# mohsij/spacecraft-pose-estimation

Hardware: AMD Instinct MI355X
Metric: poses/sec end-to-end (HRNet+PnP) at batch 256; keypoint/pose err vs ref (higher is better)
Workload: dtype bf16

## Files before the change

spacecraft-pose-estimation_amd/csrc/common.h:

```cpp
#pragma once
#include <hip/hip_runtime.h>
#include <stdint.h>
#include <stddef.h>
#include <stdarg.h>
#include <stdio.h>
#include <string>
#include <vector>
#include <string.h>

#include "../../include/scpose.h"

namespace scpose {

void set_error(const char* fmt, ...);
const char* dev_env(const char* name);
const char* last_error();

#define SCP_CHECK_HIP(expr)                                                         \
  do {                                                                              \
    hipError_t _e = (expr);                                                         \
    if (_e != hipSuccess) {                                                         \
      ::scpose::set_error("%s failed: %s (%s:%d)", #expr, hipGetErrorString(_e),    \
                          __FILE__, __LINE__);                                      \
      return SCPOSE_E_HIP;                                                          \
    }                                                                               \
  } while (0)

#define SCP_REQUIRE(cond, ...)            \
  do {                                    \
    if (!(cond)) {                        \
      ::scpose::set_error(__VA_ARGS__);   \
      return SCPOSE_E_INVALID;            \
    }                                     \
  } while (0)

#ifdef SCPOSE_DEV_BUILD
#define SCP_DBG(p, bits) ((p).dbg & (bits))
#define SCP_DBG_BUF(p) ((p).dbg_buf)
#define SCP_DEV_ONLY(x) (x)
constexpr bool kDevBuild = true;
#else
#define SCP_DBG(p, bits) (0)
#define SCP_DBG_BUF(p) (static_cast<unsigned long long*>(nullptr))
#define SCP_DEV_ONLY(x) (0)
constexpr bool kDevBuild = false;
#endif

struct LdsOptIn {
  bool done[16] = {false};
};
int32_t lds_opt_in(const void* kernel, int bytes, LdsOptIn* memo);

struct FastDiv {
  uint32_t mul, shift, add, d;
};
inline FastDiv make_fastdiv(uint32_t d) {
  FastDiv f; f.d = d ? d : 1;
  uint32_t s = 0;
  while ((2u << s) <= f.d) ++s;
  if ((f.d & (f.d - 1)) == 0) { f.mul = 0; f.add = 1; f.shift = s; }
  else { f.mul = (uint32_t)((((uint64_t)1 << (32 + s)) / f.d) + 1); f.add = 0; f.shift = s; }
  return f;
}

inline size_t align256(size_t b) { return (b + 255) & ~(size_t)255; }
struct Carve {
  uint8_t* base;
  size_t off = 0;
  template <class T>
  T* take(size_t count) {
    T* p = base ? reinterpret_cast<T*>(base + off) : nullptr;
    off += align256(count * sizeof(T));
    return p;
  }
  size_t bytes() const { return off; }
};

constexpr size_t kBufLimit = 0xfffffff0ull;
inline size_t blocked_bytes(int n, int planes, int h, int w) { return (size_t)n * planes * h * w * 16; }
inline bool fits_buf(size_t bytes) { return bytes < kBufLimit; }
inline int buf_max_frames(size_t frame_bytes, int cap = 0) {
  const int max_n = (int)(kBufLimit / frame_bytes);
  return cap > 0 && cap < max_n ? cap : max_n;
}
struct FrameRangeSwitches { int cap; bool print; };
const FrameRangeSwitches& frame_range_switches();
template <class Launch>
__attribute__((format(printf, 4, 5))) int32_t for_frame_ranges(int N, size_t frame_bytes, Launch&& launch, const char* name_fmt, ...) {
  const FrameRangeSwitches& sw = frame_range_switches();
  char name[96] = "";
  if (sw.print || !fits_buf(frame_bytes)) {
    va_list ap;
    va_start(ap, name_fmt);
    vsnprintf(name, sizeof(name), name_fmt, ap);
    va_end(ap);
  }
  SCP_REQUIRE(fits_buf(frame_bytes), "%s: one frame (%zu bytes) does not fit a 32-bit buffer descriptor", name, frame_bytes);
  const int max_n = buf_max_frames(frame_bytes, sw.cap);
  for (int n0 = 0; n0 < N; n0 += max_n) {
    const int n = N - n0 < max_n ? N - n0 : max_n;
    if (sw.print) fprintf(stderr, "%s N=%d: frames %d..%d\n", name, N, n0, n0 + n);
    const int32_t rc = launch(n0, n);
    if (rc != SCPOSE_OK) return rc;
  }
  return SCPOSE_OK;
}

struct ConvLaunch {
  const void* in;
  const void* wpk;
  const float* bias;
  const void* res;
  void* out;
  int32_t N, H, W, Ho, Wo;
  int32_t cin_planes;
  int32_t cout;
  int32_t th, tw;
  int32_t tiles_x, tiles_y;
  int32_t halo_w, halo_h;
  int32_t plane_stride;
  int32_t cp;
  int32_t nchunks;
  int32_t ksteps_full;
  int32_t n_mblk;
  int32_t relu;
  int32_t out_nchw_f32;
  int32_t store_stages;
  const void* zero16;
  int32_t items_total;
  int32_t items_per_wg;
  int32_t grid;
  int32_t lds_w, lds_x;
  int32_t lds_bias;
  int32_t nbuf_w, nbuf_x;
  int32_t tiles_total;
  int32_t nt;
  int32_t wreg_chunks;
  FastDiv fd_npix, fd_tw, fd_hp, fd_halo_w, fd_tiles_img, fd_tiles_x, fd_nmblk;
  uint32_t in_bytes, out_bytes;
  unsigned long long* dbg_buf;
  int32_t dbg;
  int32_t cu_share;
};

struct ConvConfig {
  int ks, stride;
  int mrep, nrep;
  int th, tw;
  int cp;
};

struct M32Tiling { int th = 0, tw = 0, nseg = 0, nr = 0, ps = 0, occ = 0, cp = 0, nb16 = 0; };

struct PackedConv {
  int cin, cout, ks, stride, dtype;
  int mt;
  int n_mblk;
  int cp, nchunks, ksteps_full;
  size_t wbytes;
  void* d_w = nullptr;
  float* d_bias = nullptr;
  int mrep;
  int variant = 0;
  int wm = 1;
  void* d_w1 = nullptr;
  float* d_b1 = nullptr;
  size_t w1_bytes = 0;
  int cout_pad1 = 0;
  struct TileMemo { int n = -1, ho = 0, wo = 0, cus = 0; M32Tiling t; };
  mutable TileMemo m32_memo[2];
  void* d_ws2 = nullptr;
  float* d_bs2 = nullptr;
};
bool conv_s2r_config(int cin, int cout, int stride, int* planes, int* nblk, int* g);
size_t conv_s2r_pack(const float* w, int cout, int cin, int dtype, uint16_t* dst);
void conv_s2r_pack_bias(const float* bias, int cout, float* dst);
int32_t conv_s2r_launch(const PackedConv& pc, const void* in, int N, int H, int W, int relu, void* out, hipStream_t stream);
bool conv1x1_stream_eligible(const PackedConv& pc);
int32_t conv1x1_stream_launch(const PackedConv& pc, const void* in, int N, int H, int W, const void* res, int relu,
                              void* out, hipStream_t stream);

void choose_mrep_cp(int cin, int cout, int ks, int stride, int* mrep, int* cp);
void choose_tile(int ks, int stride, int Ho, int Wo, int* nrep, int* th, int* tw);

size_t pack_conv_weights(const float* w, int cout, int cin, int ks, int mt, int cp, int dtype,
                         uint16_t* dst, int* nchunks, int* ksteps_full);

int32_t conv_upload(const float* w, const float* bias, int cout, int cin, int ks, int stride,
                    int dtype, PackedConv* pc);
void conv_free(PackedConv* pc);
int32_t conv_launch(const PackedConv& pc, const void* in, int N, int H, int W, const void* res,
                    int relu, int out_nchw_f32, void* out, hipStream_t stream, int cu_share = 0);
size_t conv_lds_bytes(const PackedConv& pc, int nrep, int th, int tw);
int plane_stride_for(int stride, int halo_h, int halo_w);
int32_t conv_launch_pipe(const PackedConv& pc, ConvLaunch& L, int nrep, int nt, int occ, hipStream_t stream);
size_t conv_pipe_lds_bytes(const PackedConv& pc, int plane_stride);
const void* conv_zero_page();
bool block_fusable(const PackedConv& c1, const PackedConv& c2);
int32_t block_launch(const PackedConv& c1, const PackedConv& c2, const void* in, int N, int H, int W, void* out,
                     hipStream_t stream);
int conv_device_cus();
unsigned long long* conv_dbg_buffer(hipStream_t stream);
void conv_dbg_set_grid(int grid);
constexpr int kMrep48 = 15;
bool conv_m32_choose(int cin, int cout, int ks, int stride, int* mr, int* wm, int* cp);
size_t pack_conv_weights_m32(const float* w, int cout, int cin, int ks, int mt, int cp, int dtype,
                             uint16_t* dst, int* nchunks, int* ksteps_full);
int32_t conv_launch_m32(const PackedConv& pc, ConvLaunch& L, hipStream_t stream);

void stem_fused_pack(const float* w1, const float* b1, const float* w2, const float* b2, int dtype, std::vector<uint16_t>* pw1,
                     std::vector<uint16_t>* pw2, std::vector<float>* pb1, std::vector<float>* pb2);
int32_t stem_fused_launch(const void* in, int in_fmt, const void* w1, const void* w2, const float* b1, const float* b2,
                          const float* mean_std, int N, int H, int W, int dtype, void* out,
                          uint32_t* sched , hipStream_t stream);

bool bottleneck_fusable(int cin, int cmid, int cout);
void bottleneck_pack(const float* w1, const float* w2, const float* w3, const float* wds, const float* b1, const float* b2, const float* b3,
                     const float* bds, int cin, int dtype,
                     std::vector<uint16_t>* pw1, std::vector<uint16_t>* pw2, std::vector<uint16_t>* pw3, std::vector<float>* pb);
int32_t bottleneck_launch(const void* in, const void* w1, const void* w2, const void* w3, const float* bias, int N, int H, int W,
                          int cin, int dtype, void* out, uint32_t* sched ,
                          hipStream_t stream);

struct FuseDownPacked {
  void* d_w = nullptr;
  float* d_b = nullptr;
  int c0 = 0, nb = 0, dtype = 0;
};
bool fuse_down_supported(int nb, int c0, int c1);
int32_t fuse_down_upload(const float* w, const float* bias, int nb, int c0, int dtype, FuseDownPacked* fd);
void fuse_down_free(FuseDownPacked* fd);
int32_t fuse_down_launch(const FuseDownPacked& fd, const void* x0, int N, int H, int W, const void* const* terms, void* y,
                         void* const* outs, hipStream_t stream);

void resnet_stem_pack(const float* w, int dtype, std::vector<uint16_t>* pw);
int32_t resnet_stem_launch(const void* in, int in_fmt, const void* w, const float* bias, const float* mean_std, int N, int H, int W,
                           int dtype, void* out, hipStream_t stream);
struct GatherClass {
  int32_t ntaps, dy[4], dx[4];
  int32_t py, px;
  long long w_off;
};
struct GatherLaunch {
  const void* in; const void* w; const float* bias; const void* res; void* out;
  int32_t N, H, W, Ho, Wo, Hb, Wb;
  int32_t cin, cout, nclass, si, so, relu;
  GatherClass cls[4];
};
struct GatherPacked {
  void* d_w = nullptr;
  float* d_bias = nullptr;
  int cin = 0, cout = 0, dtype = 0, nclass = 0, si = 1, so = 1, ks = 1;
  GatherClass cls[4];
};
int32_t deconv_upload(const float* w, const float* bias, int cout, int cin, int k, int dtype, GatherPacked* gp);
int32_t conv1x1s2_upload(const float* w, const float* bias, int cout, int cin, int dtype, GatherPacked* gp);
void gather_free(GatherPacked* gp);
void gather_out_size(const GatherPacked& gp, int H, int W, int* Ho, int* Wo);
int32_t gather_launch(const GatherPacked& gp, const void* in, int N, int H, int W, const void* res, int relu, void* out,
                      hipStream_t stream);

int32_t fuse_sum_launch(const void* const* terms, const int32_t* shifts, int nterms, int N, int C,
                        int H, int W, int dtype, void* out, hipStream_t stream);
int32_t crop_warp_launch(const uint8_t* frames, const int64_t* offsets, const int32_t* hw, const double* minv,
                         int N, int oh, int ow, int swap_rb, uint8_t* out, hipStream_t stream, const int32_t* roi = nullptr);
int events_max_width();
int32_t events_frame_bounds_launch(const int64_t* t, int64_t n, const double* starts, int F, int64_t* bounds, hipStream_t stream);
int32_t events_render_launch(const int32_t* x, const int32_t* y, const void* p, int p_bytes, const int64_t* bounds, int F,
                             int H, int W, int fs, int fold, const uint8_t* lut, const double* K, const double* dist,
                             uint8_t* frames, uint8_t* distorted, uint8_t* workspace, hipStream_t stream);
size_t events_area_workspace_bytes(int64_t n, int64_t M, int D, int h, int w);
int32_t events_area_bounds_launch(const int32_t* x, const int32_t* y, int64_t n, int64_t M, int D, int h, int w, int64_t* bounds,
                                  int64_t capacity, int64_t* count_status, uint8_t* workspace, hipStream_t stream);
int32_t events_count_bounds_launch(int64_t N, int64_t F, int64_t* bounds, hipStream_t stream);
int32_t events_bounds_midpoints_launch(const int64_t* t, const int64_t* bounds, int64_t F, double* mids, hipStream_t stream);
size_t events_csv_workspace_bytes(int64_t n_bytes);
int32_t events_csv_parse_launch(const uint8_t* data, int64_t n_bytes, int ws_mode, int swap_xy, double t_div, int64_t* t, int32_t* x,
                                int32_t* y, int8_t* p, int64_t capacity, int64_t* count_status, uint8_t* ws, hipStream_t stream);
int events_text_tile_rows();
int events_text_scan_rows();
size_t events_text_workspace_bytes(int64_t n);
int32_t events_text_measure_launch(const int64_t* t, const int32_t* x, const int32_t* y, const int8_t* p, int64_t n,
                                   int64_t* count_status, uint8_t* ws, hipStream_t stream);
int32_t events_text_emit_launch(const int64_t* t, const int32_t* x, const int32_t* y, const int8_t* p, int64_t n, int sep, int swap_xy,
                                uint8_t* out, int64_t capacity, int64_t* count_status, uint8_t* ws, hipStream_t stream);
int32_t events_aedat2_pack_launch(const int64_t* t, const int32_t* x, const int32_t* y, const int8_t* p, int64_t n, int h, int w,
                                  uint8_t* out, int64_t* count_status, hipStream_t stream);
size_t events_aedat2_unpack_workspace_bytes(int64_t n);
int32_t events_aedat2_unpack_launch(const uint8_t* records, int64_t n, int h, int w, int layout, int flip_x, int flip_y, int unwrap,
                                    double t_div, int64_t* t, int32_t* x, int32_t* y, int8_t* p, int64_t capacity, int64_t* count_status,
                                    uint8_t* ws, hipStream_t stream);
size_t events_aedat4_workspace_bytes(int64_t n_packets);
int32_t events_aedat4_measure_launch(const uint8_t* file, const int64_t* packets, int64_t n, int64_t* total_status, uint8_t* ws,
                                     hipStream_t stream);
int32_t events_aedat4_decode_launch(const uint8_t* file, const int64_t* packets, int64_t n, uint8_t* staging, int64_t staging_bytes,
                                    int verify, uint8_t* ws, hipStream_t stream);
int32_t events_aedat4_count_launch(const uint8_t* src, const int64_t* packets, int64_t n, int staged, int64_t* count_status, uint8_t* ws,
                                   hipStream_t stream);
int32_t events_aedat4_unpack_launch(const uint8_t* src, int64_t n, int h, int w, int rebase, int64_t* t, int32_t* x, int32_t* y,
                                    int8_t* p, int64_t capacity, int64_t* count_status, uint8_t* ws, hipStream_t stream);
size_t jpeg_decode_workspace_bytes(int n, int h, int w, int mode, int max_subs);
int32_t jpeg_decode_launch(const uint8_t* desc, const int32_t* segs, int64_t n_rows, const uint8_t* data, int64_t n_bytes, int n, int h,
                           int w, int mode, int max_subs, int bgr, int max_rounds, uint8_t* out, uint8_t* y_out, int32_t* status,
                           uint8_t* ws, hipStream_t stream);
int32_t jpeg_decode_crop_launch(const uint8_t* desc, const int32_t* segs, int64_t n_rows, const uint8_t* data, int64_t n_bytes, int n, int h,
                                int w, int mode, int max_subs, int bgr, int max_rounds, const double* minv, const int32_t* roi_host,
                                int out_h, int out_w, uint8_t* crops, int32_t* status, uint8_t* ws, hipStream_t stream);

size_t jpeg_encode_workspace_bytes(int n, int h, int w, int mode);
int64_t jpeg_encode_capacity_bytes(int n, int h, int w, int mode, int header_bytes);
size_t png_decode_workspace_bytes(int n, int h, int w, int channels);
int32_t png_decode_launch(const uint8_t* desc_host, const uint8_t* data, int n, int h, int w, int channels, int bgr, uint8_t* out,
                          int32_t* status, uint8_t* ws, hipStream_t stream);
int32_t png_decode_crop_launch(const uint8_t* desc_host, const uint8_t* data, int n, int h, int w, int channels, int bgr, const double* minv,
                               const int32_t* roi_host, int out_h, int out_w, uint8_t* crops, int32_t* status, uint8_t* ws,
                               hipStream_t stream);
int32_t jpeg_encode_launch(const uint8_t* frames, int n, int h, int w, int mode, int quality, const uint32_t* huff, const uint8_t* header,
                           int header_bytes, uint8_t* out, int64_t capacity, int64_t* offsets, int32_t* status, uint8_t* ws,
                           hipStream_t stream);
int32_t overlay_draw_launch(uint8_t* frames, int n, int h, int w, const int32_t* bboxes, const double* points, int j, hipStream_t stream);
size_t dvs_state_bytes(int h, int w);
size_t dvs_workspace_bytes(int h, int w, int frames, int max_iters);
int32_t dvs_init_launch(void* state, const uint8_t* frame0, double t0, int h, int w, const float* lut, double refractory_period_s,
                        hipStream_t stream);
int32_t dvs_emulate_launch(void* state, const uint8_t* frames, const double* t, int n_frames, const scpose_dvs_params& prm, float* t_s,
                           int64_t* t_us, int32_t* x, int32_t* y, int8_t* pol, int64_t capacity, int64_t* counts, uint8_t* ws,
                           hipStream_t stream);
int32_t head_gather_launch(const void* taps, const float* bias, const float* prev, int N, int J, int H, int W,
                           int K, int S, int dtype, float* out, hipStream_t stream);
int32_t heatmap_accumulate_launch(float* acc, const float* x, float div, size_t count, hipStream_t stream);
int32_t flip_merge_launch(const float* a, const float* b, const int32_t* perm, int N, int J, int H, int W, int shift,
                          float* out, hipStream_t stream);
int32_t nchw_to_blocked_launch(const float* src, int N, int C, int H, int W, int dtype, void* dst,
                               hipStream_t stream);
int32_t blocked_to_nchw_launch(const void* src, int N, int C, int H, int W, int dtype, float* dst,
                               hipStream_t stream, int Cd = -1);

void head_fused_pack(const float* w, const float* b, int J, int C, int dtype, uint16_t* wfrag, float* bias);
size_t head_fused_part_bytes(int n);
bool head_fused_supported(int nterms, int C, int J, int N, int H, int W);
int32_t head_fused_launch(const void* const* terms, const int32_t* shifts, int nterms, int N, int C, int H, int W, int J,
                          int dtype, const void* wfrag, const float* bias, float* hm, float* part_v, int32_t* part_i,
                          const float* center, const float* scale, int post_process, float* preds, hipStream_t stream);
int32_t decode_launch(const float* hm, int N, int J, int H, int W, const float* center,
                      const float* scale, int post_process, float* preds_xyc, float* coords,
                      float* maxvals, hipStream_t stream);
int32_t pnp_launch(const float* kp_xyc, const double* landmarks, const double* K,
                   const double* dist, int N, int J, double conf_thr0, int min_pts, double thr_decay,
                   int thr_iters, int max_iters, double reproj_err, double confidence, double* rot,
                   double* tvec, double* rvec, int32_t* status, hipStream_t stream, double* rows = nullptr,
                   int refine_iters = 0, unsigned long long* inliers = nullptr);

uint16_t host_f32_to_16(float f, int dtype);
float host_16_to_f32(uint16_t v, int dtype);

}
```

spacecraft-pose-estimation_amd/csrc/conv_igemm.hip:

```cpp
#include <stdio.h>
#include <stdlib.h>

#include "common.h"
#include "conv_device.h"

namespace scpose {

static int largest_divisor_leq(int n, int lim) {
  for (int d = lim < n ? lim : n; d >= 1; --d)
    if (n % d == 0) return d;
  return 1;
}

void choose_mrep_cp(int cin, int cout, int ks, int stride, int* mrep, int* cp) {
  const int mtiles = (cout + 15) / 16;
  int mr = 1;
  const int cand[5] = {6, 4, 3, 2, 1};
  for (int i = 0; i < 5; ++i)
    if (mtiles % cand[i] == 0) { mr = cand[i]; break; }
  if (mtiles >= 5 && mr == 1) mr = 4;
  *mrep = mr;
  const int planes = cin / 8;
  int lim;
  if (ks == 1) lim = 8;
  else if (stride == 2) lim = (mr >= 4) ? 2 : 4;
  else if (planes <= 6 && mtiles == mr) lim = 6;
  else if (mr >= 4) lim = 2;
  else lim = 4;
  int c = 2;
  for (int d = lim; d >= 2; d -= 2)
    if (planes % d == 0) { c = d; break; }
  *cp = c;
}

void choose_tile(int ks, int stride, int Ho, int Wo, int* nrep, int* th, int* tw) {
  const int ptmax = stride == 1 ? 256 : 128;
  int w = (Wo % 16 == 0 || Wo > 32) ? 16 : Wo;
  int h = largest_divisor_leq(Ho, ptmax / w > 0 ? ptmax / w : 1);
  const int maxhp = (stride == 1 ? 2 : 3) * 256;
  const int k2 = ks / 2;
  while (h > 1 && ((h - 1) * stride + 1 + 2 * k2) * ((w - 1) * stride + 1 + 2 * k2) > maxhp)
    h = largest_divisor_leq(Ho, h - 1);
  *th = h; *tw = w;
  *nrep = (h * w + 63) / 64;
}

uint16_t host_f32_to_16(float f, int dtype) {
  uint32_t u; memcpy(&u, &f, 4);
  if (dtype == SCPOSE_DT_BF16) {
    if ((u & 0x7fffffffu) > 0x7f800000u) return (uint16_t)((u >> 16) | 0x40);
    return (uint16_t)((u + 0x7fffu + ((u >> 16) & 1u)) >> 16);
  }
  _Float16 h = (_Float16)f;
  uint16_t b; memcpy(&b, &h, 2);
  return b;
}

float host_16_to_f32(uint16_t v, int dtype) {
  if (dtype == SCPOSE_DT_BF16) {
    uint32_t u = (uint32_t)v << 16; float f; memcpy(&f, &u, 4); return f;
  }
  _Float16 h; memcpy(&h, &v, 2);
  return (float)h;
}

static inline int conv_row_channel(int row) {
  const int q = row >> 2, reg = row & 3;
  return (q & 1) * 8 + (q >> 1) * 4 + reg;
}

size_t pack_conv_weights(const float* w, int cout, int cin, int ks, int mt, int cp, int dtype,
                         uint16_t* dst, int* nchunks_out, int* ksteps_full_out) {
  const int planes = cin / 8, kk = ks * ks;
  const int nchunks = (planes + cp - 1) / cp;
  const int ksteps_full = ((cp / 2) * kk + 1) / 2;
  const int n_mblk = (cout + mt - 1) / mt;
  const size_t chunk_elems = (size_t)ksteps_full * 4 * mt * 8;
  const size_t total = (size_t)n_mblk * nchunks * chunk_elems;
  if (nchunks_out) *nchunks_out = nchunks;
  if (ksteps_full_out) *ksteps_full_out = ksteps_full;
  if (!dst) return total * 2;
  memset(dst, 0, total * 2);
  for (int mb = 0; mb < n_mblk; ++mb)
    for (int c = 0; c < nchunks; ++c) {
      const int plane0 = c * cp;
      const int pl = (planes - plane0) < cp ? (planes - plane0) : cp;
      const int npt = (pl / 2) * kk;
      uint16_t* base = dst + ((size_t)mb * nchunks + c) * chunk_elems;
      for (int s = 0; s < (npt + 1) / 2; ++s)
        for (int q = 0; q < 4; ++q) {
          const int pt = 2 * s + (q >> 1);
          if (pt >= npt) continue;
          const int pp = pt / kk, tap = pt % kk;
          const int plane = plane0 + 2 * pp + (q & 1);
          for (int r = 0; r < mt; ++r) {
            const int co = mb * mt + (r & ~15) + conv_row_channel(r & 15);
            if (co >= cout) continue;
            uint16_t* d = base + ((size_t)(s * 4 + q) * mt + r) * 8;
            for (int j = 0; j < 8; ++j) {
              const int ci = plane * 8 + j;
              d[j] = host_f32_to_16(w[((size_t)co * cin + ci) * kk + tap], dtype);
            }
          }
        }
    }
  return total * 2;
}

int32_t conv_upload(const float* w, const float* bias, int cout, int cin, int ks, int stride,
                    int dtype, PackedConv* pc) {
  SCP_REQUIRE(ks == 1 || ks == 3, "conv: kernel size %d unsupported (1 or 3)", ks);
  SCP_REQUIRE(stride == 1 || (stride == 2 && ks == 3), "conv: stride %d with k=%d unsupported", stride, ks);
  SCP_REQUIRE(cin % 16 == 0 && cin > 0, "conv: Cin=%d must be a multiple of 16", cin);
  SCP_REQUIRE(cout > 0, "conv: Cout=%d", cout);
  SCP_REQUIRE(dtype == SCPOSE_DT_BF16 || dtype == SCPOSE_DT_F16, "conv: dtype %d", dtype);
  pc->cin = cin; pc->cout = cout; pc->ks = ks; pc->stride = stride; pc->dtype = dtype;
  std::vector<uint16_t> host;
  std::vector<float> hb;
  if (conv_m32_choose(cin, cout, ks, stride, &pc->mrep, &pc->wm, &pc->cp)) {
    pc->variant = 1;
    pc->mt = pc->mrep == kMrep48 ? 48 : 32 * pc->mrep * pc->wm;
    pc->n_mblk = (cout + pc->mt - 1) / pc->mt;
    pc->wbytes = pack_conv_weights_m32(w, cout, cin, ks, pc->mt, pc->cp, dtype, nullptr, &pc->nchunks, &pc->ksteps_full);
    host.resize(pc->wbytes / 2);
    pack_conv_weights_m32(w, cout, cin, ks, pc->mt, pc->cp, dtype, host.data(), nullptr, nullptr);
    hb.assign((size_t)pc->n_mblk * pc->mt, 0.f);
    if (bias) for (int co = 0; co < cout; ++co) hb[co] = bias[co];
  } else {
    pc->variant = 0; pc->wm = 1;
    choose_mrep_cp(cin, cout, ks, stride, &pc->mrep, &pc->cp);
    pc->mt = 16 * pc->mrep;
    pc->n_mblk = (cout + pc->mt - 1) / pc->mt;
    pc->wbytes = pack_conv_weights(w, cout, cin, ks, pc->mt, pc->cp, dtype, nullptr, &pc->nchunks,
                                   &pc->ksteps_full);
    host.resize(pc->wbytes / 2);
    pack_conv_weights(w, cout, cin, ks, pc->mt, pc->cp, dtype, host.data(), nullptr, nullptr);
    hb.assign((size_t)pc->n_mblk * pc->mt, 0.f);
    if (bias)
      for (size_t pos = 0; pos < hb.size(); ++pos) {
        const int co = (int)(pos & ~(size_t)15) + conv_row_channel((int)(pos & 15));
        if (co < cout) hb[pos] = bias[co];
      }
  }
  if (ks == 1 && stride == 1 && cout % 8 == 0 && pc->variant == 0) {
    const int planes = cin / 8, ksteps = (planes + 3) / 4, cpad = (cout + 63) / 64 * 64;
    const size_t wb = (size_t)ksteps * 4 * cpad * 16;
    const bool ks_ok = (ksteps >= 1 && ksteps <= 4) || ksteps == 6 || ksteps == 8 || ksteps == 12;
    const size_t lds1 = wb + (size_t)cpad * 4;
    if (ks_ok && lds1 <= (ksteps <= 4 ? 80 * 1024 : 156 * 1024)) {
      std::vector<uint16_t> h1(wb / 2);
      const size_t got = pack_conv_weights(w, cout, cin, 1, cpad, planes, dtype, h1.data(), nullptr, nullptr);
      SCP_REQUIRE(got == wb, "conv1x1: packed size %zu != %zu", got, wb);
      std::vector<float> b1(cpad, 0.f);
      if (bias)
        for (int pos = 0; pos < cpad; ++pos) {
          const int co = (pos & ~15) + conv_row_channel(pos & 15);
          if (co < cout) b1[pos] = bias[co];
        }
      SCP_CHECK_HIP(hipMalloc(&pc->d_w1, wb));
      SCP_CHECK_HIP(hipMalloc(&pc->d_b1, b1.size() * sizeof(float)));
      SCP_CHECK_HIP(hipMemcpy(pc->d_w1, h1.data(), wb, hipMemcpyHostToDevice));
      SCP_CHECK_HIP(hipMemcpy(pc->d_b1, b1.data(), b1.size() * sizeof(float), hipMemcpyHostToDevice));
      pc->w1_bytes = wb; pc->cout_pad1 = cpad;
    }
  }
  {
    static const char* e = dev_env("SCPOSE_S2R");
    int planes, nblk, g;
    if (ks == 3 && !(e && atoi(e) == 0) && conv_s2r_config(cin, cout, stride, &planes, &nblk, &g)) {
      std::vector<uint16_t> h2(conv_s2r_pack(w, cout, cin, dtype, nullptr) / 2);
      conv_s2r_pack(w, cout, cin, dtype, h2.data());
      std::vector<float> b2(cout);
      conv_s2r_pack_bias(bias, cout, b2.data());
      SCP_CHECK_HIP(hipMalloc(&pc->d_ws2, h2.size() * 2));
      SCP_CHECK_HIP(hipMalloc(&pc->d_bs2, b2.size() * sizeof(float)));
      SCP_CHECK_HIP(hipMemcpy(pc->d_ws2, h2.data(), h2.size() * 2, hipMemcpyHostToDevice));
      SCP_CHECK_HIP(hipMemcpy(pc->d_bs2, b2.data(), b2.size() * sizeof(float), hipMemcpyHostToDevice));
    }
  }
  SCP_REQUIRE(conv_zero_page() != nullptr, "conv: cannot allocate the zero page");
  SCP_CHECK_HIP(hipMalloc(&pc->d_w, pc->wbytes));
  SCP_CHECK_HIP(hipMalloc(&pc->d_bias, hb.size() * sizeof(float)));
  SCP_CHECK_HIP(hipMemcpy(pc->d_w, host.data(), pc->wbytes, hipMemcpyHostToDevice));
  SCP_CHECK_HIP(hipMemcpy(pc->d_bias, hb.data(), hb.size() * sizeof(float), hipMemcpyHostToDevice));
  return SCPOSE_OK;
}

void conv_free(PackedConv* pc) {
  if (pc->d_w) (void)hipFree(pc->d_w);
  if (pc->d_bias) (void)hipFree(pc->d_bias);
  if (pc->d_w1) (void)hipFree(pc->d_w1);
  if (pc->d_b1) (void)hipFree(pc->d_b1);
  if (pc->d_ws2) (void)hipFree(pc->d_ws2);
  if (pc->d_bs2) (void)hipFree(pc->d_bs2);
  pc->d_w = nullptr; pc->d_bias = nullptr; pc->d_w1 = nullptr; pc->d_b1 = nullptr; pc->d_ws2 = nullptr; pc->d_bs2 = nullptr;
}

int plane_stride_for(int stride, int halo_h, int halo_w) {
  int bytes = halo_h * halo_w * 16;
  if (stride == 1) return (bytes + 255) & ~255;
  bytes = (bytes + 31) & ~31;
  return bytes + 16;
}

size_t conv_lds_bytes(const PackedConv& pc, int nrep, int th, int tw) {
  (void)nrep;
  const int k2 = pc.ks / 2;
  const int hh = (th - 1) * pc.stride + 1 + 2 * k2, hw = (tw - 1) * pc.stride + 1 + 2 * k2;
  return 256 + (size_t)pc.ksteps_full * 4 * pc.mt * 16 +
         (size_t)pc.cp * plane_stride_for(pc.stride, hh, hw);
}

static int32_t conv_launch_range(const PackedConv& pc, const void* in, int N, int H, int W, const void* res,
                                 int relu, int out_nchw_f32, void* out, hipStream_t stream, int cu_share) {
  ConvLaunch L{};
  L.in = in; L.wpk = pc.d_w; L.bias = pc.d_bias; L.res = res; L.out = out;
  L.N = N; L.H = H; L.W = W;
  L.Ho = (H - 1) / pc.stride + 1;
  L.Wo = (W - 1) / pc.stride + 1;
  L.cin_planes = pc.cin / 8;
  L.cout = pc.cout;
  L.cu_share = cu_share;
  if (pc.d_ws2 && !res && !out_nchw_f32)
    return conv_s2r_launch(pc, in, N, H, W, relu, out, stream);
  if (pc.variant == 1) {
    SCP_REQUIRE(!out_nchw_f32, "conv m32: float32 NCHW output unsupported");
    L.relu = relu; L.out_nchw_f32 = 0;
    return conv_launch_m32(pc, L, stream);
  }
  {
    static const char* e1 = dev_env("SCPOSE_K1_STREAM");
    if (pc.d_w1 && !out_nchw_f32 && !(e1 && atoi(e1) == 0))
      return conv1x1_stream_launch(pc, in, N, H, W, res, relu, out, stream);
  }
  int nrep;
  choose_tile(pc.ks, pc.stride, L.Ho, L.Wo, &nrep, &L.th, &L.tw);
  const int k2 = pc.ks / 2;
  auto set_geometry = [&]() {
    L.tiles_x = (L.Wo + L.tw - 1) / L.tw;
    L.tiles_y = (L.Ho + L.th - 1) / L.th;
    L.halo_h = (L.th - 1) * pc.stride + 1 + 2 * k2;
    L.halo_w = (L.tw - 1) * pc.stride + 1 + 2 * k2;
    L.plane_stride = plane_stride_for(pc.stride, L.halo_h, L.halo_w);
    nrep = (L.th * L.tw + 63) / 64;
  };
  set_geometry();
  const bool resident = pc.nchunks == 1 && pc.n_mblk == 1;
  if (resident && 2 * conv_pipe_lds_bytes(pc, L.plane_stride) > 160 * 1024 && L.th % 2 == 0 && L.th * L.tw >= 128) {
    const int th0 = L.th;
    L.th /= 2;
    set_geometry();
    if (2 * conv_pipe_lds_bytes(pc, L.plane_stride) > 160 * 1024) { L.th = th0; set_geometry(); }
  }
  {
    static const char* e = dev_env("SCPOSE_TILE");
    int eth = 0, etw = 0;
    if (e && resident && pc.ks == 3 && pc.stride == 1 && sscanf(e, "%d,%d", &eth, &etw) == 2 && eth > 0 && etw > 0) {
      L.th = eth; L.tw = etw; set_geometry();
    }
  }
  int nt = 1, occ = 1;
  if (!resident && pc.ks == 3 && pc.stride == 1 && pc.mrep >= 4 && 2 * pc.mrep * nrep * 4 <= 224) nt = 2;
  if (!resident && pc.ks == 3 && pc.stride == 2 && pc.mrep >= 4 && nrep <= 2) {
    static const char* e = dev_env("SCPOSE_S2_NT");
    nt = e ? atoi(e) : 2;
  }
  if (resident && 2 * conv_pipe_lds_bytes(pc, L.plane_stride) <= 160 * 1024) occ = 2;
  static const char* e11 = dev_env("SCPOSE_K1_OCC");
  static const char* e11p = dev_env("SCPOSE_K1_MINPIX");
  if (pc.ks == 1 && !out_nchw_f32 && L.Ho * L.Wo >= (e11p ? atoi(e11p) : 4096) && !(e11 && atoi(e11) == 1) &&
      (pc.ksteps_full >= 2 || (e11 && atoi(e11) == 2))) {
    while (L.th % 2 == 0 && L.th * L.tw > 64 &&
           (2 * conv_pipe_lds_bytes(pc, L.plane_stride) > 160 * 1024 || pc.mrep * nrep * 4 > 128)) {
      L.th /= 2;
      set_geometry();
    }
    if (2 * conv_pipe_lds_bytes(pc, L.plane_stride) <= 160 * 1024 && pc.mrep * nrep * 4 <= 128) occ = 2;
  }
  L.in_bytes = (uint32_t)blocked_bytes(N, L.cin_planes, H, W);
  L.out_bytes = 0;
  L.cp = pc.cp; L.nchunks = pc.nchunks; L.ksteps_full = pc.ksteps_full;
  L.n_mblk = pc.n_mblk;
  L.relu = relu; L.out_nchw_f32 = out_nchw_f32;
  SCP_REQUIRE(L.halo_h * L.halo_w <= (pc.stride == 1 ? 2 : 3) * 256, "conv: halo %dx%d too large",
              L.halo_h, L.halo_w);
  SCP_REQUIRE((pc.ksteps_full + 1) * 4 <= 64, "conv: k-offset table overflow (%d ksteps)", pc.ksteps_full);
  return conv_launch_pipe(pc, L, nrep, nt, occ, stream);
}

int32_t conv_launch(const PackedConv& pc, const void* in, int N, int H, int W, const void* res,
                    int relu, int out_nchw_f32, void* out, hipStream_t stream, int cu_share) {
  SCP_REQUIRE(N > 0 && H > 0 && W > 0, "conv: bad shape N=%d H=%d W=%d", N, H, W);
  SCP_REQUIRE(out_nchw_f32 || pc.cout % 8 == 0, "conv: blocked output needs Cout%%8==0 (Cout=%d)", pc.cout);
  const int Ho = (H - 1) / pc.stride + 1, Wo = (W - 1) / pc.stride + 1;
  const size_t in_frame = blocked_bytes(1, pc.cin / 8, H, W), blk_frame = blocked_bytes(1, (pc.cout + 7) / 8, Ho, Wo);
  const size_t out_frame = out_nchw_f32 ? (size_t)pc.cout * Ho * Wo * 4 : blk_frame;
  return for_frame_ranges(N, in_frame > blk_frame ? in_frame : blk_frame, [&](int n0, int n) -> int32_t {
    return conv_launch_range(pc, static_cast<const char*>(in) + (size_t)n0 * in_frame, n, H, W,
                             res ? static_cast<const char*>(res) + (size_t)n0 * blk_frame : nullptr, relu, out_nchw_f32,
                             static_cast<char*>(out) + (size_t)n0 * out_frame, stream, cu_share);
  }, "conv %d->%d k%d s%d %dx%d", pc.cin, pc.cout, pc.ks, pc.stride, H, W);
}

}
```

Before: 9861.

## Add persistent stride-2 3x3 conv kernel for 384-channel outputs

Adds a new specialized stride-2 3x3 convolution kernel for cin 192/256 to cout 384 layers (variant m32 path). It runs one persistent workgroup per CU over output tiles, double-buffers input halo tiles in LDS via DMA, and streams a custom-packed weight layout from global memory with a three-deep register pipeline feeding 32x32 MFMAs. It is dispatched only when the tile count covers all CUs, falling back to the existing m32 path otherwise. The aim is to cut halo load overhead and improve MFMA utilization for the HRNet downsampling layers, at the cost of extra weight memory and a new code path.

```diff
diff --git a/spacecraft-pose-estimation_amd/csrc/common.h b/spacecraft-pose-estimation_amd/csrc/common.h
--- a/spacecraft-pose-estimation_amd/csrc/common.h
+++ b/spacecraft-pose-estimation_amd/csrc/common.h
@@ -171,11 +171,16 @@
   mutable TileMemo m32_memo[2];
   void* d_ws2 = nullptr;
   float* d_bs2 = nullptr;
+  void* d_ws2w = nullptr;
 };
 bool conv_s2r_config(int cin, int cout, int stride, int* planes, int* nblk, int* g);
 size_t conv_s2r_pack(const float* w, int cout, int cin, int dtype, uint16_t* dst);
 void conv_s2r_pack_bias(const float* bias, int cout, float* dst);
 int32_t conv_s2r_launch(const PackedConv& pc, const void* in, int N, int H, int W, int relu, void* out, hipStream_t stream);
+bool conv_s2w_config(int cin, int cout, int stride);
+bool conv_s2w_takes(int N, int Ho, int Wo);
+size_t conv_s2w_pack(const float* w, int cout, int cin, int dtype, uint16_t* dst);
+int32_t conv_s2w_launch(const PackedConv& pc, const void* in, int N, int H, int W, int relu, void* out, hipStream_t stream);
 bool conv1x1_stream_eligible(const PackedConv& pc);
 int32_t conv1x1_stream_launch(const PackedConv& pc, const void* in, int N, int H, int W, const void* res, int relu,
                               void* out, hipStream_t stream);
diff --git a/spacecraft-pose-estimation_amd/csrc/conv_igemm.hip b/spacecraft-pose-estimation_amd/csrc/conv_igemm.hip
--- a/spacecraft-pose-estimation_amd/csrc/conv_igemm.hip
+++ b/spacecraft-pose-estimation_amd/csrc/conv_igemm.hip
@@ -178,6 +178,15 @@
       SCP_CHECK_HIP(hipMemcpy(pc->d_bs2, b2.data(), b2.size() * sizeof(float), hipMemcpyHostToDevice));
     }
   }
+  {
+    static const char* e = dev_env("SCPOSE_S2W");
+    if (ks == 3 && pc->variant == 1 && !(e && atoi(e) == 0) && conv_s2w_config(cin, cout, stride)) {
+      std::vector<uint16_t> h3(conv_s2w_pack(w, cout, cin, dtype, nullptr) / 2);
+      conv_s2w_pack(w, cout, cin, dtype, h3.data());
+      SCP_CHECK_HIP(hipMalloc(&pc->d_ws2w, h3.size() * 2));
+      SCP_CHECK_HIP(hipMemcpy(pc->d_ws2w, h3.data(), h3.size() * 2, hipMemcpyHostToDevice));
+    }
+  }
   SCP_REQUIRE(conv_zero_page() != nullptr, "conv: cannot allocate the zero page");
   SCP_CHECK_HIP(hipMalloc(&pc->d_w, pc->wbytes));
   SCP_CHECK_HIP(hipMalloc(&pc->d_bias, hb.size() * sizeof(float)));
@@ -193,7 +202,8 @@
   if (pc->d_b1) (void)hipFree(pc->d_b1);
   if (pc->d_ws2) (void)hipFree(pc->d_ws2);
   if (pc->d_bs2) (void)hipFree(pc->d_bs2);
-  pc->d_w = nullptr; pc->d_bias = nullptr; pc->d_w1 = nullptr; pc->d_b1 = nullptr; pc->d_ws2 = nullptr; pc->d_bs2 = nullptr;
+  if (pc->d_ws2w) (void)hipFree(pc->d_ws2w);
+  pc->d_w = nullptr; pc->d_bias = nullptr; pc->d_w1 = nullptr; pc->d_b1 = nullptr; pc->d_ws2 = nullptr; pc->d_bs2 = nullptr; pc->d_ws2w = nullptr;
 }
 
 int plane_stride_for(int stride, int halo_h, int halo_w) {
@@ -223,6 +233,8 @@
   L.cu_share = cu_share;
   if (pc.d_ws2 && !res && !out_nchw_f32)
     return conv_s2r_launch(pc, in, N, H, W, relu, out, stream);
+  if (pc.d_ws2w && !res && !out_nchw_f32 && conv_s2w_takes(N, L.Ho, L.Wo))
+    return conv_s2w_launch(pc, in, N, H, W, relu, out, stream);
   if (pc.variant == 1) {
     SCP_REQUIRE(!out_nchw_f32, "conv m32: float32 NCHW output unsupported");
     L.relu = relu; L.out_nchw_f32 = 0;
diff --git a/spacecraft-pose-estimation_amd/csrc/conv_s2w.hip b/spacecraft-pose-estimation_amd/csrc/conv_s2w.hip
--- /dev/null
+++ b/spacecraft-pose-estimation_amd/csrc/conv_s2w.hip
@@ -0,0 +1,253 @@
+#include "common.h"
+#include "conv_device.h"
+#include "conv_m32_kernel.h"
+#include "conv_pipe_kernel.h"
+
+namespace scpose {
+
+namespace {
+
+constexpr int kRG = 4, kPG = 2, kMR = 3, kNR = 3;
+constexpr int kSlots = kPG * kNR * 32;
+constexpr int kRowBlocks = kRG * kMR;
+constexpr int kMaxPieces = 2;
+
+struct S2wLaunch {
+  const void* in;
+  const void* w;
+  const float* bias;
+  void* out;
+  uint32_t in_bytes, out_bytes, w_bytes;
+  int32_t N, H, W, Ho, Wo, cin_planes, relu;
+  int32_t th, tw, hw, hp, pitch_bytes;
+  int32_t tiles_x, tiles_y, tiles_total, tiles_per_wg, grid;
+  FastDiv fd_tiles_img, fd_tiles_x, fd_tw, fd_hw;
+};
+
+__device__ __forceinline__ int s2w_fdiv(int n, const FastDiv& f) {
+  return (int)((__umulhi((uint32_t)n, f.mul) + (uint32_t)n * f.add) >> f.shift);
+}
+
+}
+
+template <int DT>
+__global__ __launch_bounds__(512) void conv_s2w_kernel(const S2wLaunch p) {
+  extern __shared__ __attribute__((aligned(16))) char smem[];
+  typedef typename DtOf<DT>::type T;
+  typedef typename FragOf<T>::type frag_t;
+
+  const int tid = threadIdx.x, lane = tid & 63, wave = __builtin_amdgcn_readfirstlane(tid >> 6);
+  const int half = lane >> 5, r = lane & 31;
+  const int rg = wave & (kRG - 1), pg = wave / kRG;
+  const int HW = p.H * p.W;
+  const int nst = p.cin_planes >> 1;
+  const int npix = p.th * p.tw;
+  const int tiles_per_img = p.tiles_x * p.tiles_y;
+  const int XB = 2 * p.pitch_bytes;
+
+  int hy[kMaxPieces], hx[kMaxPieces];
+#pragma unroll
+  for (int i = 0; i < kMaxPieces; ++i) {
+    const int slot = (wave + 8 * i) * 64 + lane;
+    hy[i] = slot < p.hp ? s2w_fdiv(slot, p.fd_hw) : -1;
+    hx[i] = slot < p.hp ? slot - hy[i] * p.hw : 0;
+  }
+  int pixoff[kNR];
+#pragma unroll
+  for (int n = 0; n < kNR; ++n) {
+    const int pidx = (pg * kNR + n) * 32 + r;
+    const int py = s2w_fdiv(pidx, p.fd_tw), px = pidx - py * p.tw;
+    pixoff[n] = (pidx < npix ? ((2 * py) * p.hw + 2 * px) * 16 : 0) + half * p.pitch_bytes;
+  }
+
+  const int wg = xcd_remap(blockIdx.x, p.grid);
+  const int t_begin = wg * p.tiles_per_wg;
+  const int t_end = min(p.tiles_total, t_begin + p.tiles_per_wg);
+  if (t_begin >= t_end) return;
+  auto decode = [&](int t, int& img, int& oy0, int& ox0) {
+    img = s2w_fdiv(t, p.fd_tiles_img);
+    const int rem = t - img * tiles_per_img;
+    const int ty = s2w_fdiv(rem, p.fd_tiles_x);
+    oy0 = ty * p.th; ox0 = (rem - ty * p.tiles_x) * p.tw;
+  };
+  const buf_rsrc_t rs_in = make_buf(p.in, p.in_bytes), rs_out = make_buf(p.out, p.out_bytes), rs_w = make_buf(p.w, p.w_bytes);
+
+  auto issue_x = [&](int t, int s, int b) {
+    int img, oy0, ox0;
+    decode(t, img, oy0, ox0);
+    char* xl = smem + b * XB;
+#pragma unroll
+    for (int i = 0; i < kMaxPieces; ++i) {
+      const int iy = 2 * oy0 - 1 + hy[i], ix = 2 * ox0 - 1 + hx[i];
+      const bool ok = iy >= 0 && iy < p.H && ix >= 0 && ix < p.W;
+      const uint32_t voff = ok ? (uint32_t)(img * p.cin_planes * HW + iy * p.W + ix) * 16u : BUF_OOB;
+      if (hy[i] >= 0) {
+        dma16_buf(rs_in, voff, (uint32_t)((2 * s) * HW) * 16u, xl + (wave + 8 * i) * 1024);
+        dma16_buf(rs_in, voff, (uint32_t)((2 * s + 1) * HW) * 16u, xl + p.pitch_bytes + (wave + 8 * i) * 1024);
+      }
+    }
+  };
+  auto load_a = [&](int s, int tap, frag_t* a) {
+    const uint32_t soff = (uint32_t)(((s * 9 + tap) * kRowBlocks + rg * kMR) * 1024);
+#pragma unroll
+    for (int m = 0; m < kMR; ++m) a[m] = __builtin_bit_cast(frag_t, load16_buf(rs_w, (uint32_t)lane * 16u, soff + (uint32_t)m * 1024u));
+  };
+
+  frag_t af[3][kMR];
+  issue_x(t_begin, 0, 0);
+  load_a(0, 0, af[0]);
+  load_a(0, 1, af[1]);
+  asm volatile("s_waitcnt vmcnt(0)" ::: "memory");
+  __syncthreads();
+
+  const size_t HoWo = (size_t)p.Ho * p.Wo;
+  const int cout_planes = kRowBlocks * 4;
+  const uint32_t relu_floor = p.relu ? 0u : 0x80008000u;
+  f32x16 acc[kMR][kNR];
+  int buf = 0;
+  for (int t = t_begin; t < t_end; ++t) {
+#pragma unroll
+    for (int m = 0; m < kMR; ++m) {
+      const float* bp = p.bias + (rg * kMR + m) * 32 + 4 * half;
+#pragma unroll
+      for (int g = 0; g < 4; ++g) {
+        const float4 b4 = *reinterpret_cast<const float4*>(bp + 8 * g);
+#pragma unroll
+        for (int n = 0; n < kNR; ++n) { acc[m][n][4 * g] = b4.x; acc[m][n][4 * g + 1] = b4.y; acc[m][n][4 * g + 2] = b4.z; acc[m][n][4 * g + 3] = b4.w; }
+      }
+    }
+    for (int s = 0; s < nst; ++s, buf ^= 1) {
+      const bool last = s + 1 == nst;
+      if (!last) issue_x(t, s + 1, buf ^ 1);
+      else if (t + 1 < t_end) issue_x(t + 1, 0, buf ^ 1);
+      const int sn = last ? 0 : s + 1;
+      const char* xl = smem + buf * XB;
+      frag_t bf[2][kNR];
+#pragma unroll
+      for (int n = 0; n < kNR; ++n) bf[0][n] = *reinterpret_cast<const frag_t*>(xl + pixoff[n]);
+#pragma unroll
+      for (int tap = 0; tap < 9; ++tap) {
+        if (tap + 1 < 9) {
+          const int ky = (tap + 1) / 3, kx = (tap + 1) - 3 * ky;
+#pragma unroll
+          for (int n = 0; n < kNR; ++n) bf[(tap + 1) & 1][n] = *reinterpret_cast<const frag_t*>(xl + pixoff[n] + (ky * p.hw + kx) * 16);
+        }
+        if (tap + 2 < 9) load_a(s, tap + 2, af[(tap + 2) % 3]);
+        else load_a(sn, tap + 2 - 9, af[(tap + 2) % 3]);
+        __builtin_amdgcn_sched_barrier(0);
+#pragma unroll
+        for (int n = 0; n < kNR; ++n)
+#pragma unroll
+          for (int m = 0; m < kMR; ++m) acc[m][n] = mfma32<T>(af[tap % 3][m], bf[tap & 1][n], acc[m][n]);
+        __builtin_amdgcn_sched_barrier(0);
+      }
+      if (last) {
+        int img, oy0, ox0;
+        decode(t, img, oy0, ox0);
+#pragma unroll
+        for (int n = 0; n < kNR; ++n) {
+          int pidx = (pg * kNR + n) * 32 + r;
+          asm volatile("" : "+v"(pidx));
+          const int py = s2w_fdiv(pidx, p.fd_tw), px = pidx - py * p.tw;
+          const int oy = oy0 + py, ox = ox0 + px;
+          const bool ok = pidx < npix && oy < p.Ho && ox < p.Wo;
+          const uint32_t pix = (uint32_t)(((size_t)img * cout_planes * HoWo + (size_t)oy * p.Wo + ox) * 16);
+#pragma unroll
+          for (int m = 0; m < kMR; ++m)
+#pragma unroll
+            for (int g = 0; g < 2; ++g) {
+              uint32_t a[2], b[2];
+              a[0] = relu2_16(pack2<T>(acc[m][n][8 * g + 0], acc[m][n][8 * g + 1]), relu_floor);
+              a[1] = relu2_16(pack2<T>(acc[m][n][8 * g + 2], acc[m][n][8 * g + 3]), relu_floor);
+              b[0] = relu2_16(pack2<T>(acc[m][n][8 * g + 4], acc[m][n][8 * g + 5]), relu_floor);
+              b[1] = relu2_16(pack2<T>(acc[m][n][8 * g + 6], acc[m][n][8 * g + 7]), relu_floor);
+#pragma unroll
+              for (int jj = 0; jj < 2; ++jj) {
+                const auto sw = __builtin_amdgcn_permlane32_swap(a[jj], b[jj], false, false);
+                a[jj] = sw[0]; b[jj] = sw[1];
+              }
+              const int plane = (rg * kMR + m) * 4 + 2 * g + half;
+              const uint32_t voff = ok ? pix + (uint32_t)((size_t)plane * HoWo * 16) : BUF_OOB;
+              store16_buf(rs_out, voff, 0u, u32x4{a[0], a[1], b[0], b[1]});
+            }
+        }
+      }
+      asm volatile("s_waitcnt vmcnt(0) lgkmcnt(0)\n\ts_barrier" ::: "memory");
+    }
+  }
+}
+
+bool conv_s2w_config(int cin, int cout, int stride) {
+  return stride == 2 && cout == 32 * kRowBlocks && (cin == 192 || cin == 256);
+}
+
+size_t conv_s2w_pack(const float* w, int cout, int cin, int dtype, uint16_t* dst) {
+  const int npp = cin / 16, nrb = cout / 32;
+  const size_t total = (size_t)npp * 9 * nrb * 2 * 32 * 8;
+  if (!dst) return total * 2;
+  for (int pp = 0; pp < npp; ++pp)
+    for (int tap = 0; tap < 9; ++tap)
+      for (int rb = 0; rb < nrb; ++rb)
+        for (int kg = 0; kg < 2; ++kg)
+          for (int r = 0; r < 32; ++r) {
+            const int co = rb * 32 + r, plane = 2 * pp + kg;
+            uint16_t* d = dst + (((((size_t)pp * 9 + tap) * nrb + rb) * 2 + kg) * 32 + r) * 8;
+            for (int j = 0; j < 8; ++j) d[j] = host_f32_to_16(w[((size_t)co * cin + plane * 8 + j) * 9 + tap], dtype);
+          }
+  return total * 2;
+}
+
+static void s2w_tile(int Ho, int Wo, int* th, int* tw) {
+  *tw = Wo < 16 ? Wo : 16;
+  *th = kSlots / *tw;
+  if (*th > Ho) *th = Ho;
+  while (*th > 1 && (2 * *th + 1) * (2 * *tw + 1) > kMaxPieces * 8 * 64) --*th;
+}
+
+bool conv_s2w_takes(int N, int Ho, int Wo) {
+  static const char* e = dev_env("SCPOSE_S2W");
+  if (e && atoi(e) == 2) return true;
+  int th, tw;
+  s2w_tile(Ho, Wo, &th, &tw);
+  const long tiles = (long)N * ((Wo + tw - 1) / tw) * ((Ho + th - 1) / th);
+  return tiles >= conv_device_cus();
+}
+
+template <int DT>
+static int32_t s2w_launch_one(const S2wLaunch& L, hipStream_t st) {
+  auto kern = conv_s2w_kernel<DT>;
+  const size_t lds = 4 * (size_t)L.pitch_bytes;
+  static LdsOptIn big;
+  { const int32_t rc = lds_opt_in(reinterpret_cast<const void*>(kern), (int)lds, &big); if (rc != SCPOSE_OK) return rc; }
+  hipLaunchKernelGGL(kern, dim3(L.grid), dim3(512), lds, st, L);
+  SCP_CHECK_HIP(hipGetLastError());
+  return SCPOSE_OK;
+}
+
+int32_t conv_s2w_launch(const PackedConv& pc, const void* in, int N, int H, int W, int relu, void* out, hipStream_t stream) {
+  SCP_REQUIRE(conv_s2w_config(pc.cin, pc.cout, pc.stride) && pc.d_ws2w, "conv s2w: %d->%d not eligible", pc.cin, pc.cout);
+  S2wLaunch L{};
+  L.in = in; L.w = pc.d_ws2w; L.bias = pc.d_bias; L.out = out;
+  L.N = N; L.H = H; L.W = W; L.Ho = (H - 1) / 2 + 1; L.Wo = (W - 1) / 2 + 1;
+  L.cin_planes = pc.cin / 8; L.relu = relu;
+  L.in_bytes = (uint32_t)((size_t)N * L.cin_planes * H * W * 16);
+  L.out_bytes = (uint32_t)((size_t)N * (pc.cout / 8) * L.Ho * L.Wo * 16);
+  L.w_bytes = (uint32_t)conv_s2w_pack(nullptr, pc.cout, pc.cin, pc.dtype, nullptr);
+  s2w_tile(L.Ho, L.Wo, &L.th, &L.tw);
+  L.hw = 2 * L.tw + 1;
+  L.hp = (2 * L.th + 1) * L.hw;
+  SCP_REQUIRE(L.th * L.tw <= kSlots && L.hp <= kMaxPieces * 8 * 64, "conv s2w: tile %d x %d does not fit", L.th, L.tw);
+  L.pitch_bytes = (L.hp | 1) * 16;
+  L.tiles_x = (L.Wo + L.tw - 1) / L.tw; L.tiles_y = (L.Ho + L.th - 1) / L.th;
+  L.tiles_total = N * L.tiles_x * L.tiles_y;
+  L.fd_tiles_img = make_fastdiv(L.tiles_x * L.tiles_y); L.fd_tiles_x = make_fastdiv(L.tiles_x);
+  L.fd_tw = make_fastdiv(L.tw); L.fd_hw = make_fastdiv(L.hw);
+  int grid = conv_device_cus();
+  if (grid > L.tiles_total) grid = L.tiles_total;
+  L.tiles_per_wg = (L.tiles_total + grid - 1) / grid;
+  L.grid = (L.tiles_total + L.tiles_per_wg - 1) / L.tiles_per_wg;
+  if (pc.dtype == SCPOSE_DT_BF16) return s2w_launch_one<0>(L, stream);
+  return s2w_launch_one<1>(L, stream);
+}
+
+}
```

Result: no change. 9941, median of 6 (+0.8%).
